# onecodex/needletail

Measured on AMD Instinct MI355X. Metric: Gbases/s canonical k=21 on 150 bp FASTQ; % HBM-read roofline at 1/2/4/8 GPU, higher is better.
Workload: dtype u64; 1 GPU; configs[1]: synthetic FASTQ 10M x 150 bp, k=21 canonical k-mers (normalize -> reverse_complement -> canonical_kmers), reduce mode, device-resident batch; reads_total=10000000, reads_this_gpu=10000000, read_len=150, k=21, seed=0x5eed0002, outputs=n_total,n_fwd,n_rc,4096-bin prefix histogram,sum64,xor64, parallelism=single GPU, rccl_ranks=0, devices_visible=1

## Files before the change

include/needletail_amd.h:

```cpp
#ifndef NEEDLETAIL_AMD_H
#define NEEDLETAIL_AMD_H

#include <stddef.h>
#include <stdint.h>

#ifdef __cplusplus
extern "C" {
#endif

#define NTK_ABI_VERSION 4

enum {
    NTK_OK = 0,
    NTK_ERR_BAD_K = 1,
    NTK_ERR_BAD_ARG = 2,
    NTK_ERR_HIP = 3,
    NTK_ERR_NO_DEVICE = 4,
    NTK_ERR_CAPACITY = 5,
    NTK_ERR_UNSUPPORTED = 6,
    NTK_ERR_NOMEM = 7,
    NTK_ERR_PARSE = 8,
    NTK_ERR_RCCL = 9,
    NTK_EOF = 100
};
// ... 35 lines not shown
    uint64_t hist[NTK_HIST_BINS];
    uint64_t n_undigested;
} ntk_result;
#define NTK_ACC_N_TOTAL 0
#define NTK_ACC_N_FWD 1
#define NTK_ACC_N_RC 2
#define NTK_ACC_SUM 3
#define NTK_ACC_XOR 4
#define NTK_ACC_UNDIGESTED 5
#define NTK_ACC_REDONE 6
#define NTK_ACC_HIST 8
#define NTK_ACC_XOR_BITS (8 + NTK_HIST_BINS)
#define NTK_ACC_WORDS (8 + NTK_HIST_BINS + 64)

typedef struct ntk_ctx ntk_ctx;
int ntk_ctx_create(int device, ntk_ctx **out);
int ntk_ctx_create_on_stream(int device, void *hip_stream, ntk_ctx **out);
void ntk_ctx_destroy(ntk_ctx *ctx);
int ntk_ctx_synchronize(ntk_ctx *ctx);
int ntk_ctx_stream(ntk_ctx *ctx, int *device, void **hip_stream);
int ntk_ctx_set_launch(ntk_ctx *ctx, int blocks, int threads_per_block);
enum { NTK_OPT_COMPAT_CHUNK_BYTES = 1, NTK_OPT_MINIMIZER_CHUNK_BYTES = 2, NTK_OPT_MINIMIZER_ROUTE = 3, NTK_OPT_COMPAT_PACK_THREADS = 4,
       NTK_OPT_COPY_STREAMS = 5, NTK_OPT_BATCH_WAIT_POLL_US = 6, NTK_OPT_GZ_INMEM_LIMIT_BYTES = 7, NTK_OPT_GZ_STREAM_WINDOW_BYTES = 8,
       NTK_OPT_PIPE_STATS = 9 };
#define NTK_POLL_BLOCK 0xFFFFFFFFu
#define NTK_ROUTE_NO_REGFUSED 1u
#define NTK_ROUTE_NO_GENERIC 2u
#define NTK_ROUTE_NO_F64 4u
#define NTK_ROUTE_NO_SPECULATION 8u
int ntk_ctx_set_option(ntk_ctx *ctx, int option, uint64_t value);
int ntk_ctx_get_option(ntk_ctx *ctx, int option, uint64_t *value);
int ntk_ctx_enable_timing(ntk_ctx *ctx, int on);
int ntk_ctx_scan_time_ms(ntk_ctx *ctx, double *total_ms, uint64_t *launches);

typedef struct ntk_comm ntk_comm;
#define NTK_COMM_ID_BYTES 128
int ntk_comm_init_all(ntk_ctx *const *ctxs, int n, ntk_comm **out);
int ntk_comm_unique_id(uint8_t id[NTK_COMM_ID_BYTES]);
int ntk_comm_init_rank(ntk_ctx *ctx, int n_ranks, int rank, const uint8_t id[NTK_COMM_ID_BYTES], ntk_comm **out);
int ntk_comm_size(const ntk_comm *comm);
int ntk_allreduce_accumulators(ntk_comm *comm);
int ntk_comm_allreduce_time_ms(ntk_comm *comm, double *total_ms, uint64_t *calls);
void ntk_comm_destroy(ntk_comm *comm);

int ntk_accum_reset(ntk_ctx *ctx);
int ntk_reduce_device(ntk_ctx *ctx, const uint8_t *d_seq, uint64_t n_bytes, const ntk_params *p);
int ntk_reduce_device_quality(ntk_ctx *ctx, const uint8_t *d_seq, const uint8_t *d_qual, uint64_t n_bytes,
// ... 108 lines not shown
```

needletail_amd/_lib.py:

```python
from __future__ import annotations

import ctypes as C
import os

_HERE = os.path.dirname(os.path.abspath(__file__))
LIB_PATH = os.environ.get("NEEDLETAIL_AMD_LIB") or os.path.join(_HERE, "libneedletail_amd.so")

NTK_OK = 0
PATH_BYTES_CANONICAL, PATH_BITS, PATH_BITS_CANONICAL = 0, 1, 2
PRE_NONE, PRE_STRIP_RETURNS, PRE_NORMALIZE, PRE_NORMALIZE_IUPAC = 0, 1, 2, 3
HIST_BINS = 4096
ACC_N_TOTAL, ACC_N_FWD, ACC_N_RC, ACC_SUM, ACC_XOR, ACC_HIST = 0, 1, 2, 3, 4, 8
ACC_UNDIGESTED, ACC_REDONE = 5, 6
ACC_XOR_BITS, ACC_WORDS = 8 + 4096, 8 + 4096 + 64
OPT_COMPAT_CHUNK_BYTES, OPT_MINIMIZER_CHUNK_BYTES, OPT_MINIMIZER_ROUTE, OPT_COMPAT_PACK_THREADS, OPT_COPY_STREAMS = 1, 2, 3, 4, 5
OPT_BATCH_WAIT_POLL_US, OPT_GZ_INMEM_LIMIT_BYTES, OPT_GZ_STREAM_WINDOW_BYTES, OPT_PIPE_STATS = 6, 7, 8, 9
POLL_BLOCK = 0xFFFFFFFF
ROUTE_NO_REGFUSED, ROUTE_NO_GENERIC, ROUTE_NO_F64, ROUTE_NO_SPECULATION = 1, 2, 4, 8
ROUTE_TWO_PASS = ROUTE_NO_REGFUSED | ROUTE_NO_GENERIC

SYMBOLS = [
    "ntk_strerror", "ntk_last_hip_error", "ntk_last_rccl_error", "ntk_abi_version", "ntk_device_count",
    "ntk_comm_init_all", "ntk_comm_unique_id", "ntk_comm_init_rank", "ntk_comm_size", "ntk_allreduce_accumulators", "ntk_comm_allreduce_time_ms", "ntk_comm_destroy",
    "ntk_ctx_create", "ntk_ctx_create_on_stream", "ntk_ctx_destroy", "ntk_ctx_synchronize", "ntk_ctx_stream",
    "ntk_ctx_set_launch", "ntk_ctx_set_option", "ntk_ctx_get_option", "ntk_ctx_enable_timing", "ntk_ctx_scan_time_ms",
    "ntk_accum_reset", "ntk_reduce_device", "ntk_reduce_device_quality", "ntk_accum_read", "ntk_accum_device_ptr", "ntk_accum_bind_device",
    "ntk_materialize_device", "ntk_materialize_device_quality",
    "ntk_batch_acquire", "ntk_batch_append", "ntk_batch_append_quality", "ntk_batch_buffers", "ntk_batch_submit", "ntk_batch_wait",
    "ntk_batch_release",
    "ntk_normalize", "ntk_strip_returns", "ntk_reverse_complement", "ntk_canonical_kmers", "ntk_bit_kmers", "ntk_canonical_kmers_batch", "ntk_bit_kmers_batch", "ntk_pinned_alloc", "ntk_pinned_free",
    "ntk_canonical_kmers_batch_planes", "ntk_bit_kmers_batch_planes", "ntk_ctx_trim", "ntk_minimizer_batch",
    "ntk_synth_reads_device", "ntk_reverse_complement_records_device",
    "ntk_reader_open_file", "ntk_reader_open_memory", "ntk_reader_next", "ntk_reader_error", "ntk_reader_position", "ntk_reader_close",
    "ntk_scan_reader", "ntk_scan_buffer_parallel", "ntk_scan_file_parallel", "ntk_fastx_split_points", "ntk_gunzip", "ntk_gunzip_free", "ntk_scan_file_info",
    "ntk_minimizers_reduce_device", "ntk_minimizer", "ntk_canonical", "ntk_bit_minimizers", "ntk_quality_mask", "ntk_bit_canonical",
]


class Params(C.Structure):
# ... 158 lines not shown
```

needletail_amd/csrc/ntk_api.hip:

```cpp
#include "../../include/needletail_amd.h"

#include <hip/hip_runtime.h>
#include <rccl/rccl.h>
#include <dlfcn.h>
#include <time.h>

#include <cstdlib>
#include <cstring>
#include <map>
#include <mutex>
#include <new>
#include <utility>
#include <thread>
#include <algorithm>
#include <vector>

#include "ntk_kernels.hpp"

using namespace ntk;

const void *ntk_pick_scan2(int k, bool tie_rc, bool accept_u);
const void *ntk_pick_scan2_q(int k, bool canonical, bool tie_rc, bool accept_u);
const void *ntk_pick_scan2_min_a(int k, int w, bool tie_rc, bool accept_u, bool quality);
const void *ntk_pick_scan2_min_b(int k, int w, bool tie_rc, bool accept_u, bool quality);
// ... 72 lines not shown

struct ntk_ctx {
    int device = 0;
    hipStream_t stream = nullptr;
    hipStream_t copy_stream = nullptr;
    hipStream_t copy_stream2 = nullptr;
    uint32_t copy_streams = 2, copy_rr = 0;
    hipStream_t down_stream = nullptr;
    bool owns_stream = false;
    int n_cu = 256;
    int launch_blocks = 0, launch_threads = 0;
    uint64_t *d_acc = nullptr;
    uint64_t *d_acc_own = nullptr;
    uint32_t *d_part_hist = nullptr;
    uint32_t *d_work = nullptr;
    bool work_dirty = true;
    uint32_t *d_lower = nullptr;
    uint32_t lower_idx = 0;
    uint64_t minimizer_chunk = (uint64_t)256 << 20;
    uint64_t compat_chunk = (uint64_t)16 << 20;
    uint32_t route_off = 0;
    uint32_t pack_threads = 8;
    uint64_t wait_poll_us = 50;
    uint64_t gz_limit = 0, gz_window = 0, pipe_stats = 0;
    uint64_t *d_part_scalars = nullptr;
    int part_blocks = 0;
    uint16_t *d_lut = nullptr;
    Scratch scratch[6];
    CompatBank bank[3];
    void *h_pinned = nullptr;
    bool timing = false;
    std::vector<hipEvent_t> ev_free;
    std::vector<std::pair<hipEvent_t, hipEvent_t>> ev_used;
    std::map<std::pair<const void *, int>, int> occupancy;
    std::map<const void *, int> auto_threads;
    std::mutex pool_mu;
    std::vector<ntk_batch *> pool;
    uint64_t pool_bytes = 0;
};

struct ntk_batch {
    uint8_t *h_seq = nullptr;
    uint64_t *h_off = nullptr;
    uint8_t *d_seq = nullptr;
    uint8_t *h_qual = nullptr, *d_qual = nullptr;
    bool has_qual = false;
// ... 240 lines not shown
int launch_tile_scan(ntk_ctx *c, const TileScan &s, ScanArgs &a, bool zero_first)
{
    int per_cu = 0, rc = resident_blocks(c, s.fn, s.threads, s.lds, s.max_per_cu, &per_cu);
    if (rc) return rc;
    const uint64_t blocks_max = block_cap(c, per_cu), waves_per_block = (uint64_t)s.threads / 64;
    const uint64_t tile_slots = 64 - (uint64_t)s.halo_lanes, tile_stride = tile_slots * 16, n = a.n_bytes;
    const int blocks_raw = s.speculate ? raw_bytes_blocks(c, n) : 0;
    a.n_tiles = tile_count(n, tile_slots);
    a.work_counters = c->d_work;
    a.zero_words = NTK_ACC_WORDS;
    for (uint64_t tb = 0; tb < a.n_tiles; tb += kMaxTilesPerLaunch) {
        const uint64_t te = tb + kMaxTilesPerLaunch < a.n_tiles ? tb + kMaxTilesPerLaunch : a.n_tiles;
        const uint64_t tiles = te - tb;
        uint64_t chunk = tiles / (blocks_max * waves_per_block * 4);
        chunk = chunk < 1 ? 1 : (chunk > s.max_chunk ? s.max_chunk : chunk);
        const uint64_t want_blocks = (tiles + chunk * waves_per_block - 1) / (chunk * waves_per_block);
        const int blocks = (int)(want_blocks < blocks_max ? want_blocks : blocks_max);
        a.tile_begin = tb; a.tile_end = te;
        const uint64_t first_tail = n / tile_stride;
        a.tail_tile_rel = first_tail < tb ? 0u : (first_tail - tb > 0xFFFFFFFEull ? 0xFFFFFFFFu : (uint32_t)(first_tail - tb));
        a.n_shards = blocks < kMaxShards ? (uint32_t)blocks : (uint32_t)kMaxShards;
        a.tiles_per_shard = (uint32_t)((tiles + a.n_shards - 1) / a.n_shards);
        a.chunk_tiles = (uint32_t)chunk;
        a.zero_acc = zero_first ? c->d_acc : nullptr;
        zero_first = false;
        if (c->work_dirty) HIPCHK(hipMemsetAsync(c->d_work, 0, kMaxShards * 64, c->stream));
        c->work_dirty = true;
        if (s.reduce) {
            if ((rc = ensure_partials(c, blocks > blocks_raw ? blocks : blocks_raw))) return rc;
            a.part_hist = c->d_part_hist; a.part_scalars = c->d_part_scalars;
        }
        Fold fold;
        fold.rearm_shards = a.n_shards;
        if (s.speculate) {
            const FlagPair f = next_flag(c);
            a.lower_flag = f.flag; a.lower_flag_next = f.next;
            fold.alt_flag = f.flag; fold.alt_rows = blocks_raw;
        }
        TimedSpan span;
        if ((rc = span.begin(c))) return rc;
        void *kargs[] = {(void *)&a};
        HIPCHK(hipLaunchKernel(s.fn, dim3(blocks), dim3(s.threads), kargs, s.lds, c->stream));
        if (s.speculate) {
            launch_raw_bytes(c, false, blocks_raw, a.seq, n, a.k, fold.alt_flag, false, a.qual, s.cutoff);
            HIPCHK(hipGetLastError());
        }
// ... 241 lines not shown
    return NTK_OK;
}

int ntk_ctx_set_launch(ntk_ctx *c, int blocks, int threads)
{
    if (!c || blocks < 0 || threads < 0 || threads > 1024 || (threads & 63)) return NTK_ERR_BAD_ARG;
    c->launch_blocks = blocks; c->launch_threads = threads;
    return NTK_OK;
}

int ntk_ctx_get_option(ntk_ctx *c, int option, uint64_t *value)
{
    if (!c || !value) return NTK_ERR_BAD_ARG;
    switch (option) {
    case NTK_OPT_COMPAT_CHUNK_BYTES: *value = c->compat_chunk; return NTK_OK;
    case NTK_OPT_MINIMIZER_CHUNK_BYTES: *value = c->minimizer_chunk; return NTK_OK;
    case NTK_OPT_MINIMIZER_ROUTE: *value = c->route_off; return NTK_OK;
    case NTK_OPT_COMPAT_PACK_THREADS: *value = c->pack_threads; return NTK_OK;
    case NTK_OPT_COPY_STREAMS: *value = c->copy_streams; return NTK_OK;
    case NTK_OPT_BATCH_WAIT_POLL_US: *value = c->wait_poll_us ? c->wait_poll_us : NTK_POLL_BLOCK; return NTK_OK;
    case NTK_OPT_GZ_INMEM_LIMIT_BYTES: *value = c->gz_limit; return NTK_OK;
    case NTK_OPT_GZ_STREAM_WINDOW_BYTES: *value = c->gz_window; return NTK_OK;
    case NTK_OPT_PIPE_STATS: *value = c->pipe_stats; return NTK_OK;
    default: return NTK_ERR_BAD_ARG;
    }
}

int ntk_ctx_set_option(ntk_ctx *c, int option, uint64_t value)
{
    if (!c) return NTK_ERR_BAD_ARG;
    switch (option) {
    case NTK_OPT_COMPAT_CHUNK_BYTES:
        c->compat_chunk = value == 0 ? ((uint64_t)16 << 20) : (value < 64 ? 64 : value);
        return NTK_OK;
    case NTK_OPT_MINIMIZER_CHUNK_BYTES:
        if (value && value < 4096) return NTK_ERR_BAD_ARG;
        c->minimizer_chunk = value == 0 ? ((uint64_t)256 << 20) : (value & ~(uint64_t)4095);
        return NTK_OK;
    case NTK_OPT_MINIMIZER_ROUTE:
        if (value & ~(uint64_t)(NTK_ROUTE_NO_REGFUSED | NTK_ROUTE_NO_GENERIC | NTK_ROUTE_NO_F64 | NTK_ROUTE_NO_SPECULATION)) return NTK_ERR_BAD_ARG;
        c->route_off = (uint32_t)value;
        return NTK_OK;
    case NTK_OPT_BATCH_WAIT_POLL_US:
        c->wait_poll_us = value == 0 ? 50 : (value == NTK_POLL_BLOCK ? 0 : (value > 10000000 ? 10000000 : value));
        return NTK_OK;
    case NTK_OPT_GZ_INMEM_LIMIT_BYTES: c->gz_limit = value; return NTK_OK;
// ... 1208 lines not shown
```

needletail_amd/csrc/ntk_kernels.hpp:

```cpp
#pragma once
#include <hip/hip_runtime.h>
#include <stdint.h>
#include <type_traits>

#include "ntk_tile.hpp"

#if !defined(NTK_KBENCH) && (defined(NTK_ABL_LOADSONLY) || defined(NTK_ABL_FLOOR) || defined(NTK_ABL_NOLDS) || defined(NTK_ABL_NODIGEST) || \
                             defined(NTK_ABL_NOEXEC) || defined(NTK_ABL_NOSDWA) || defined(NTK_ABL_NOMASKALG) || defined(NTK_V_CLOCKS) || \
                             defined(NTK_X_CMPFIRST) || defined(NTK_X_TWOPHASE) || defined(NTK_X_MFMASUM) || defined(NTK_X_SELOUT) || defined(NTK_X_PREFETCH2) || defined(NTK_X_FASTSTART) || defined(NTK_ABL_HALFIMPORTS))
#error "NTK_ABL_* / NTK_X_* / NTK_V_CLOCKS are kernel-bench switches: build with -DNTK_KBENCH (tools/build_kbench.sh), never into the library"
#endif

namespace ntk {

typedef uint32_t u32x4 __attribute__((ext_vector_type(4)));

constexpr int kDppWaveShr1 = 0x138;
struct DevXL {
    __device__ __forceinline__ uint32_t prev_and(int s, uint32_t x, uint32_t mask) const { return prev(s, x) & mask; }
    __device__ __forceinline__ uint32_t prev_auto(uint32_t x) const { return prev(0, x); }
    __device__ __forceinline__ uint32_t prev(int, uint32_t x) const
    {
        return (uint32_t)__builtin_amdgcn_mov_dpp((int)x, kDppWaveShr1, 0xf, 0xf, true);
    }
    __device__ __forceinline__ uint32_t prev_add(int, uint32_t x, uint32_t c) const
    {
        uint32_t r;
        asm("s_nop 1\n v_add_u32_dpp %0, %1, %2 wave_shr:1 row_mask:0xf bank_mask:0xf bound_ctrl:1" : "=v"(r) : "v"(x), "v"(c));
        return r;
    }
    __device__ __forceinline__ uint32_t select_prev(int, bool take, uint32_t a, uint32_t b) const
    {
// ... 562 lines not shown
#define NTK_SV2_MINWAVES 1
#endif
template <int K, bool TIE_RC, bool ACCEPT_U, bool QM = false, int HB = 12, int W = 0, bool FWD = false>
__global__ __launch_bounds__(1024, NTK_SV2_MINWAVES) void scan2_kernel(ScanArgs a)
{
    static_assert(K >= 1 && K <= 32 && (HB == 12 || HB == 14), "sv2 covers 1 <= k <= 32");
    static_assert(W == 0 || Sv2MinFused<K, W>::value, "fused minimizers: see ntk_tile.hpp");
    static_assert(W == 0 || K <= 16 || Sv2Light<K, HB>::value, "fused minimizers sum the lo word only: the cell must cover the bits above it");
    constexpr bool WORD = K <= 16;
    constexpr bool LIGHT = Sv2Light<K, HB>::value && !WORD;
    constexpr int kCells = 1 << HB;
    using Geo = Sv2Geom<(W ? K + W - 1 : K)>;
    constexpr uint32_t kStride = Geo::kStride, kHaloB = Geo::kHaloBytes;
    struct Lds { uint32_t hist[kCells]; uint64_t red[16 * 6]; };
    __shared__ Lds L;
    uint32_t *const s_hist = L.hist;
    uint64_t *const s_red = L.red;
    if ((uint32_t)(uintptr_t)&L.hist[0] != 0u) __builtin_trap();

#ifdef NTK_V_CLOCKS
    const uint64_t dbg_c0 = clock64(), dbg_w0 = wall_clock64();
    uint32_t dbg_tiles = 0;
#endif
#ifndef NTK_X_FASTSTART
    if (a.zero_acc && blockIdx.x == 0)
        for (uint32_t i = threadIdx.x; i < a.zero_words; i += blockDim.x) a.zero_acc[i] = 0;
    for (int i = threadIdx.x; i < kCells; i += blockDim.x) s_hist[i] = 0;
    __syncthreads();

#endif
    const uint32_t lane = threadIdx.x & 63u;
    const uint32_t wave = __builtin_amdgcn_readfirstlane(threadIdx.x >> 6);
    const uint32_t shard = blockIdx.x % a.n_shards;
    const uint32_t launch_tiles = (uint32_t)(a.tile_end - a.tile_begin);
    const uint32_t shard_begin = shard * a.tiles_per_shard;
    uint32_t shard_end = shard_begin + a.tiles_per_shard;
    if (shard_end > launch_tiles) shard_end = launch_tiles;
    uint32_t *ctr = a.work_counters + shard * 16;
    const uint32_t shard_tiles = shard_begin < shard_end ? shard_end - shard_begin : 0u;
#ifdef NTK_X_FASTSTART
    uint32_t next = 0;
    if (lane == 0) next = atomicAdd(ctr, a.chunk_tiles);
    if (a.zero_acc && blockIdx.x == 0)
        for (uint32_t i = threadIdx.x; i < a.zero_words; i += blockDim.x) a.zero_acc[i] = 0;
    for (int i = threadIdx.x; i < kCells / 4; i += blockDim.x) reinterpret_cast<u32x4 *>(s_hist)[i] = u32x4{0u, 0u, 0u, 0u};
    __syncthreads();
#endif
    constexpr bool SPEC = TIE_RC && !ACCEPT_U && W == 0 && !FWD;
    uint32_t lc = 0;
    if (SPEC && a.lower_flag_next && blockIdx.x == 0 && threadIdx.x == 0) *a.lower_flag_next = 0;
    DevXL xl;
    DevMasks2<K, HB> mp;
    NoSink sink;
    mp.rep = lane & (uint32_t)(DevMasks2<K, HB>::kWordCopies - 1);
#ifdef NTK_X_MFMASUM
    { const int sel = 1 << (8 * (lane & 3)); mp.msel = {sel, sel, sel, sel}; }
#endif

#ifndef NTK_X_FASTSTART
    uint32_t next = 0;
    if (lane == 0) next = atomicAdd(ctr, a.chunk_tiles);
#endif
    next = __builtin_amdgcn_readfirstlane(next);
#ifdef NTK_X_GUIDED
    uint32_t c_cur = a.chunk_tiles;
    const uint32_t shard_waves2 = 2u * ((gridDim.x + a.n_shards - 1) / a.n_shards) * (blockDim.x >> 6);
#endif
    while (next < shard_tiles) {
        const uint32_t r0 = shard_begin + next;
#ifdef NTK_X_GUIDED
        uint32_t r1 = r0 + c_cur;
        if (r1 > shard_end) r1 = shard_end;
        {
            const uint32_t done = next + c_cur < shard_tiles ? next + c_cur : shard_tiles;
            uint32_t c = (shard_tiles - done) / shard_waves2;
            c = c < 2u ? 2u : (c > a.chunk_tiles ? a.chunk_tiles : c);
            c_cur = c;
            if (lane == 0) next = atomicAdd(ctr, c);
        }
#else
        uint32_t r1 = r0 + a.chunk_tiles;
        if (r1 > shard_end) r1 = shard_end;
        if (lane == 0) next = atomicAdd(ctr, a.chunk_tiles);
#endif
        const uint64_t t0 = a.tile_begin + r0;
        const uint64_t run_byte = t0 * kStride;
        const uint32_t halo = t0 ? kHaloB : 0u;
        const uint64_t cbase = (uint64_t)a.seq + run_byte - halo;
        uint64_t rem = ((a.n_bytes + 15) & ~(uint64_t)15) - (run_byte - halo);
        if (rem > 0xFFFFFF00ull) rem = 0xFFFFFF00ull;
        const uint32_t blo = __builtin_amdgcn_readfirstlane((uint32_t)cbase);
        const uint32_t bhi = __builtin_amdgcn_readfirstlane((uint32_t)(cbase >> 32));
        const uint32_t nrec = __builtin_amdgcn_readfirstlane((uint32_t)rem);
        __amdgpu_buffer_rsrc_t rs = __builtin_amdgcn_make_buffer_rsrc((void *)(((uint64_t)bhi << 32) | blo), 0, nrec, 0x00020000);
        __amdgpu_buffer_rsrc_t rq = rs;
        if constexpr (QM) {
            const uint64_t qbase = (uint64_t)a.qual + run_byte - halo;
            const uint32_t qlo = __builtin_amdgcn_readfirstlane((uint32_t)qbase);
            const uint32_t qhi = __builtin_amdgcn_readfirstlane((uint32_t)(qbase >> 32));
            rq = __builtin_amdgcn_make_buffer_rsrc((void *)(((uint64_t)qhi << 32) | qlo), 0, nrec, 0x00020000);
        }
        uint32_t voff = lane * 16u - (kHaloB - halo);
        uint64_t tile_byte = run_byte;
#ifdef NTK_ABL_FLOOR
        auto load_tile = [&](uint32_t off) { (void)rs; return u32x4{off, off, off, off}; };
#else
        auto load_tile = [&](uint32_t off) { return __builtin_amdgcn_raw_buffer_load_b128(rs, off, 0, 0); };
#endif
        auto load_qual = [&](uint32_t off) { return __builtin_amdgcn_raw_buffer_load_b128(rq, off, 0, 0); };
#ifdef NTK_ABL_FLOOR
        uint32_t fl_code = lane * 0x9E3779B9u + r0, fl_rcode = ~fl_code, fl_step = 0x85EBCA6Bu + lane;
        asm volatile("" : "+v"(fl_step));
#pragma unroll
        for (int i = 0; i < 16; i++) { mp.VA[i] = ~3ull; mp.VB[i] = ~0ull; }
#endif
        auto process = [&](const u32x4 &t, const u32x4 &q, uint32_t r, auto &&after_encode) {
            const bool tail = r >= a.tail_tile_rel;
            Raw16 raw{t.x, t.y, t.z, t.w};
            if constexpr (SPEC && !QM) {
                if (tail) lc |= or_of_input_bytes(raw, (int64_t)a.n_bytes - ((int64_t)tile_byte - (int64_t)kHaloB + lane * 16));
                else lc = bitop3<0xFE>(bitop3<0xFE>(lc, t.x, t.y), t.z, t.w);
            }
            if constexpr (QM) raw = quality_break16(raw, Raw16{q.x, q.y, q.z, q.w}, a.q_add, a.q_sel);
            if constexpr (SPEC && QM) {
                if (tail) lc |= or_of_input_bytes(lower_watch16(raw), (int64_t)a.n_bytes - ((int64_t)tile_byte - (int64_t)kHaloB + lane * 16));
                else lc = lower_watch_or(lower_watch_or(lower_watch_or(lower_watch_or(lc, raw.x), raw.y), raw.z), raw.w);
            }
#ifdef NTK_ABL_LOADSONLY
            mp.xlo ^= raw.x ^ raw.y ^ raw.z ^ raw.w; (void)tail;
            after_encode();
#elif defined(NTK_ABL_FLOOR)
            (void)tail; (void)raw;
            after_encode();
            fl_code += fl_step; fl_rcode += fl_code;
            lane_tile_sv2<TIE_RC, K>(sink, xl, mp, fl_code, fl_rcode);
#else
            const EncSV2 en = encode16_sv2<ACCEPT_U>(raw);
            mp.template compute<(W ? K + W - 1 : K)>(en, tail, (int64_t)tile_byte - (int64_t)kHaloB + lane * 16, a.n_bytes);
            after_encode();
            if constexpr (W > 0) lane_tile_sv2_min<TIE_RC, K, W>(sink, xl, mp, en.code, en.rcode);
            else if constexpr (WORD) lane_tile_sv2w<TIE_RC, K, FWD>(sink, xl, mp, en.code, en.rcode);
            else if constexpr (FWD) lane_tile_sv2_fwd<K>(sink, xl, mp, en.code);
            else lane_tile_sv2<TIE_RC, K>(sink, xl, mp, en.code, en.rcode);
#endif
            voff += kStride; tile_byte += kStride;
#ifdef NTK_V_CLOCKS
            dbg_tiles++;
#endif
        };
        u32x4 ta = load_tile(voff), qa = ta;
        if constexpr (QM) qa = load_qual(voff);
#ifdef NTK_X_PREFETCH2
        u32x4 tb = ta;
        if (r0 + 1 < r1) tb = load_tile(voff + kStride);
        for (uint32_t r = r0; r < r1; r += 2) {
            process(ta, qa, r, [&] { if (r + 2 < r1) ta = load_tile(voff + 2 * kStride); });
            if (r + 1 < r1) process(tb, qa, r + 1, [&] { if (r + 3 < r1) tb = load_tile(voff + 2 * kStride); });
        }
#else
        for (uint32_t r = r0; r < r1; r++)
            process(ta, qa, r, [&] {
                if (r + 1 < r1) { ta = load_tile(voff + kStride); if constexpr (QM) qa = load_qual(voff + kStride); }
            });
#endif
        next = __builtin_amdgcn_readfirstlane(next);
    }

#ifdef NTK_V_CLOCKS
    if ((threadIdx.x & 63) == 0 && a.values) {
        uint32_t hwid, xcc;
        asm volatile("s_getreg_b32 %0, hwreg(HW_REG_HW_ID)" : "=s"(hwid));
        asm volatile("s_getreg_b32 %0, hwreg(HW_REG_XCC_ID)" : "=s"(xcc));
        const size_t w = (size_t)blockIdx.x * (blockDim.x >> 6) + (threadIdx.x >> 6);
        a.values[w * 4 + 0] = dbg_w0; a.values[w * 4 + 1] = wall_clock64();
        a.values[w * 4 + 2] = ((clock64() - dbg_c0) & 0xFFFFFFFFFFull) | ((uint64_t)dbg_tiles << 40); a.values[w * 4 + 3] = ((uint64_t)xcc << 32) | hwid;
    }
#endif
    if constexpr (SPEC)
        if (a.lower_flag && __builtin_amdgcn_ballot_w64((lc & 0x20202020u) != 0u) != 0ull && lane == 0) atomicOr(a.lower_flag, 1u);
    asm volatile("s_waitcnt lgkmcnt(0)" ::: "memory");
    uint64_t sum = mp.sum + mp.sum2 + ((uint64_t)mp.sumh << 32);
#ifdef NTK_X_MFMASUM
    if ((lane & 15) < 4) sum += (uint64_t)(int64_t)(mp.macc.x + mp.macc.y + mp.macc.z + mp.macc.w) << (8 * (lane & 3));
#endif
    uint64_t xr = (WORD || LIGHT) ? (uint64_t)mp.xlo : ((uint64_t)mp.xh << 32) | mp.xlo, nf, nv = 0;
    uint64_t shi = 0, xf = 0;
    uint32_t *ph = a.part_hist + (size_t)blockIdx.x * kHistBins;
    nf = lane == 0 ? mp.nf_s : 0u;
    if constexpr (W > 0) nf = mp.nf_bits;
    __syncthreads();
    constexpr int HBE = HB;
    for (int c = threadIdx.x; c < kHistBins; c += blockDim.x) {
        uint32_t tot = 0;
        if constexpr (K <= 6) {
            if (c < (1 << (2 * K)))
                for (int r = 0; r < DevMasks2<K, HB>::kWordCopies; r++) tot += s_hist[(r << (2 * K)) + c];
        } else
#pragma unroll
        for (int q = 0; q < kCells / kHistBins; q++) {
            const uint32_t f = c * (kCells / kHistBins) + q, h = s_hist[f];
            tot += h;
            if constexpr (LIGHT) {
                const uint32_t pfx = f >> (HB - HBE);
                shi += (uint64_t)(pfx >> (32 + HBE - 2 * K)) * h;
                xf ^= (h & 1u) ? pfx : 0u;
            }
        }
        ph[c] = tot; nv += tot;
    }
    if constexpr (LIGHT) {
        constexpr uint32_t low_mask = 2 * K - HBE >= 32 ? 0xFFFFFFFFu : ((1u << ((2 * K - HBE) & 31)) - 1u);
        sum += shi << 32;
        xr = (xf << (2 * K - HBE)) | (uint64_t)(mp.xlo & low_mask);
    }
#pragma unroll
    for (int o = 32; o > 0; o >>= 1) {
        sum += __shfl_xor(sum, o, 64);
        xr ^= __shfl_xor(xr, o, 64);
        nf += __shfl_xor(nf, o, 64);
        nv += __shfl_xor(nv, o, 64);
    }
    if (lane == 0) { s_red[wave * 4 + 0] = nv; s_red[wave * 4 + 1] = nf; s_red[wave * 4 + 2] = sum; s_red[wave * 4 + 3] = xr; }
    __syncthreads();
    if (threadIdx.x == 0) {
        uint64_t tv = 0, tf = 0, ts = 0, tx = 0;
        for (uint32_t w = 0; w < (blockDim.x >> 6); w++) {
            tv += s_red[w * 4 + 0]; tf += s_red[w * 4 + 1]; ts += s_red[w * 4 + 2]; tx ^= s_red[w * 4 + 3];
        }
        uint64_t *ps = a.part_scalars + (size_t)blockIdx.x * 4;
        if constexpr (W > 0 && !TIE_RC) tf = tv - tf;
        if constexpr (FWD) tf = tv;
        if constexpr (WORD && K < 16 && W == 0) { ts >>= 32 - 2 * K; tx >>= 32 - 2 * K; }
        ps[0] = tv; ps[1] = tf; ps[2] = ts; ps[3] = tx;
    }
}

#ifndef NTK_SCAN_TEMPLATES_ONLY
#ifndef NTK_MINGEN_WAVES_F64
#define NTK_MINGEN_WAVES_F64 4
#endif
#ifndef NTK_MINGEN_WAVES_G
#define NTK_MINGEN_WAVES_G 4
#endif
constexpr int min_gen_waves(bool f64) { return f64 ? NTK_MINGEN_WAVES_F64 : NTK_MINGEN_WAVES_G; }
constexpr int min_gen_threads(bool f64) { return min_gen_waves(f64) == 3 ? 768 : 512; }
struct DevMinOut {
    uint64_t sum = 0, sum2 = 0;
    uint32_t sumh = 0, xh = 0;
    uint32_t xlo = 0, nfb = 0, one = 1;
    template <bool WIDE>
    __device__ __forceinline__ void region(const uint64_t *V, const uint32_t (&off)[4], const uint32_t (&lo)[4], const uint32_t (&hi)[4],
                                           const uint32_t (&sb)[4])
    {
        uint64_t sd;
#define NTK_M_POS(i, ACC, W)                                                \
        "s_mov_b64 exec, %[m" #i "]\n"                                      \
// ... 154 lines not shown
                if (light) { shi += (uint64_t)(f >> (46u - 2u * kk)) * h; xf ^= (h & 1u) ? f : 0u; }
            }
        ph[c] = tot;
    }
    if (light) {
        const uint32_t low_bits = 2u * kk - 14u;
        sum += shi << 32;
        xr = (xf << low_bits) | (low_bits >= 32u ? xr : (xr & ((1ull << low_bits) - 1ull)));
    }
#pragma unroll
    for (int o = 32; o > 0; o >>= 1) {
        sum += __shfl_xor(sum, o, 64); xr ^= __shfl_xor(xr, o, 64); nf += __shfl_xor(nf, o, 64); nv += __shfl_xor(nv, o, 64);
    }
    if (lane == 0) { s_red[wave * 4 + 0] = nv; s_red[wave * 4 + 1] = nf; s_red[wave * 4 + 2] = sum; s_red[wave * 4 + 3] = xr; }
    __syncthreads();
    if (threadIdx.x == 0) {
        uint64_t tv = 0, tf = 0, ts = 0, tx = 0;
        for (uint32_t w = 0; w < (blockDim.x >> 6); w++) { tv += s_red[w * 4 + 0]; tf += s_red[w * 4 + 1]; ts += s_red[w * 4 + 2]; tx ^= s_red[w * 4 + 3]; }
        uint64_t *ps = a.part_scalars + (size_t)blockIdx.x * 4;
        ps[0] = tv; ps[1] = tf; ps[2] = ts; ps[3] = tx;
    }
}

constexpr int kFoldThreads = 256, kFoldBinGroups = kHistBins / kFoldThreads, kFoldRowGroups = 32;
constexpr int kFoldBlocks = kFoldBinGroups * kFoldRowGroups + 1;
__global__ __launch_bounds__(kFoldThreads) void fold_kernel(const uint32_t *part_hist, const uint64_t *part_scalars, int nblocks,
                                                            uint64_t *acc, uint32_t *work_counters = nullptr, int n_counters = 8,
                                                            const uint32_t *select = nullptr, int nblocks_alt = 0, int undigested = 0)
{
    if (select && *select) nblocks = nblocks_alt;
    if (blockIdx.x < kFoldBinGroups * kFoldRowGroups) {
        const int bin = (blockIdx.x % kFoldBinGroups) * kFoldThreads + threadIdx.x;
        uint64_t s = 0;
#pragma unroll 8
        for (int b = blockIdx.x / kFoldBinGroups; b < nblocks; b += kFoldRowGroups) s += part_hist[(size_t)b * kHistBins + bin];
        if (s) atomicAdd((unsigned long long *)&acc[8 + bin], (unsigned long long)s);
        return;
    }
    __shared__ uint64_t s_red[kFoldThreads / 64][4];
    if (work_counters)
        for (int i = threadIdx.x; i < n_counters; i += kFoldThreads) work_counters[i * 16] = 0;
    uint64_t tv = 0, tf = 0, ts = 0, tx = 0;
    for (int b = threadIdx.x; b < nblocks; b += kFoldThreads) {
        tv += part_scalars[b * 4 + 0]; tf += part_scalars[b * 4 + 1];
        ts += part_scalars[b * 4 + 2]; tx ^= part_scalars[b * 4 + 3];
    }
#pragma unroll
    for (int o = 32; o > 0; o >>= 1) {
        tv += __shfl_xor(tv, o, 64); tf += __shfl_xor(tf, o, 64); ts += __shfl_xor(ts, o, 64); tx ^= __shfl_xor(tx, o, 64);
    }
    if ((threadIdx.x & 63) == 0) { s_red[threadIdx.x >> 6][0] = tv; s_red[threadIdx.x >> 6][1] = tf; s_red[threadIdx.x >> 6][2] = ts; s_red[threadIdx.x >> 6][3] = tx; }
    __syncthreads();
    if (threadIdx.x < 64) {
        tv = tf = ts = tx = 0;
        for (int w = 0; w < kFoldThreads / 64; w++) { tv += s_red[w][0]; tf += s_red[w][1]; ts += s_red[w][2]; tx ^= s_red[w][3]; }
        if (threadIdx.x == 0) {
            acc[0] += tv; acc[1] += tf; acc[2] += tv - tf; acc[3] += ts; acc[4] ^= tx;
            if (undigested) acc[5] += tv;
            if (select && *select) acc[6] += 1;
        }
        acc[8 + kHistBins + threadIdx.x] += (tx >> threadIdx.x) & 1;
    }
}


template <int THREADS, class T>
__device__ __forceinline__ T block_exclusive_scan(T v, T *s_wave, T *total = nullptr)
{
    T x = v;
#pragma unroll
    for (int o = 1; o < 64; o <<= 1) {
        const T y = __shfl_up(x, o, 64);
        if ((int)(threadIdx.x & 63) >= o) x += y;
    }
    __syncthreads();
    if ((threadIdx.x & 63) == 63) s_wave[threadIdx.x >> 6] = x;
    __syncthreads();
    T wave_off = 0, all = 0;
#pragma unroll
    for (int w = 0; w < THREADS / 64; w++) {
        const T t = s_wave[w];
        if (w < (int)(threadIdx.x >> 6)) wave_off += t;
        all += t;
    }
// ... 901 lines not shown
```

Measured before the change: 3231 Gbases/s.

## Statically assign first scan chunks per wave, defer LDS zeroing, restructure fold kernel

Each wave now takes its first chunk from a fixed offset based on its shard rank instead of an atomic, and later atomic pulls are offset by a pull base. The tile load for the first chunk is issued before the LDS histogram is zeroed, so the two can overlap. The histogram epilogue reads LDS with 128-bit loads and writes partials with relaxed atomic stores. The fold kernel uses fewer row groups, keeps 16 rows of 128-bit loads in flight per wave, combines waves through LDS, and reads the scalar accumulators early. Together these aim to cut startup and atomic contention and raise memory-level parallelism in the fold, at the cost of more complex work-distribution logic that must stay consistent with the counter reset.

Result: no change. 3256 Gbases/s (median of 2 runs) (+0.8%).

```diff
diff --git a/include/needletail_amd.h b/include/needletail_amd.h
--- a/include/needletail_amd.h
+++ b/include/needletail_amd.h
@@ -81,7 +81,7 @@
 int ntk_ctx_set_launch(ntk_ctx *ctx, int blocks, int threads_per_block);
 enum { NTK_OPT_COMPAT_CHUNK_BYTES = 1, NTK_OPT_MINIMIZER_CHUNK_BYTES = 2, NTK_OPT_MINIMIZER_ROUTE = 3, NTK_OPT_COMPAT_PACK_THREADS = 4,
        NTK_OPT_COPY_STREAMS = 5, NTK_OPT_BATCH_WAIT_POLL_US = 6, NTK_OPT_GZ_INMEM_LIMIT_BYTES = 7, NTK_OPT_GZ_STREAM_WINDOW_BYTES = 8,
-       NTK_OPT_PIPE_STATS = 9 };
+       NTK_OPT_PIPE_STATS = 9, NTK_OPT_LAST_SCAN_WAVES = 10, NTK_OPT_LAST_SCAN_CHUNK_TILES = 11 };
 #define NTK_POLL_BLOCK 0xFFFFFFFFu
 #define NTK_ROUTE_NO_REGFUSED 1u
 #define NTK_ROUTE_NO_GENERIC 2u
diff --git a/needletail_amd/_lib.py b/needletail_amd/_lib.py
--- a/needletail_amd/_lib.py
+++ b/needletail_amd/_lib.py
@@ -15,6 +15,7 @@
 ACC_XOR_BITS, ACC_WORDS = 8 + 4096, 8 + 4096 + 64
 OPT_COMPAT_CHUNK_BYTES, OPT_MINIMIZER_CHUNK_BYTES, OPT_MINIMIZER_ROUTE, OPT_COMPAT_PACK_THREADS, OPT_COPY_STREAMS = 1, 2, 3, 4, 5
 OPT_BATCH_WAIT_POLL_US, OPT_GZ_INMEM_LIMIT_BYTES, OPT_GZ_STREAM_WINDOW_BYTES, OPT_PIPE_STATS = 6, 7, 8, 9
+OPT_LAST_SCAN_WAVES, OPT_LAST_SCAN_CHUNK_TILES = 10, 11
 POLL_BLOCK = 0xFFFFFFFF
 ROUTE_NO_REGFUSED, ROUTE_NO_GENERIC, ROUTE_NO_F64, ROUTE_NO_SPECULATION = 1, 2, 4, 8
 ROUTE_TWO_PASS = ROUTE_NO_REGFUSED | ROUTE_NO_GENERIC
diff --git a/needletail_amd/csrc/ntk_api.hip b/needletail_amd/csrc/ntk_api.hip
--- a/needletail_amd/csrc/ntk_api.hip
+++ b/needletail_amd/csrc/ntk_api.hip
@@ -118,6 +118,7 @@
     uint32_t route_off = 0;
     uint32_t pack_threads = 8;
     uint64_t wait_poll_us = 50;
+    uint64_t last_scan_waves = 0, last_scan_chunk = 0;
     uint64_t gz_limit = 0, gz_window = 0, pipe_stats = 0;
     uint64_t *d_part_scalars = nullptr;
     int part_blocks = 0;
@@ -404,6 +405,7 @@
         a.n_shards = blocks < kMaxShards ? (uint32_t)blocks : (uint32_t)kMaxShards;
         a.tiles_per_shard = (uint32_t)((tiles + a.n_shards - 1) / a.n_shards);
         a.chunk_tiles = (uint32_t)chunk;
+        c->last_scan_waves = (uint64_t)blocks * waves_per_block; c->last_scan_chunk = chunk;
         a.zero_acc = zero_first ? c->d_acc : nullptr;
         zero_first = false;
         if (c->work_dirty) HIPCHK(hipMemsetAsync(c->d_work, 0, kMaxShards * 64, c->stream));
@@ -691,6 +693,8 @@
     case NTK_OPT_GZ_INMEM_LIMIT_BYTES: *value = c->gz_limit; return NTK_OK;
     case NTK_OPT_GZ_STREAM_WINDOW_BYTES: *value = c->gz_window; return NTK_OK;
     case NTK_OPT_PIPE_STATS: *value = c->pipe_stats; return NTK_OK;
+    case NTK_OPT_LAST_SCAN_WAVES: *value = c->last_scan_waves; return NTK_OK;
+    case NTK_OPT_LAST_SCAN_CHUNK_TILES: *value = c->last_scan_chunk; return NTK_OK;
     default: return NTK_ERR_BAD_ARG;
     }
 }
diff --git a/needletail_amd/csrc/ntk_kernels.hpp b/needletail_amd/csrc/ntk_kernels.hpp
--- a/needletail_amd/csrc/ntk_kernels.hpp
+++ b/needletail_amd/csrc/ntk_kernels.hpp
@@ -7,7 +7,7 @@
 
 #if !defined(NTK_KBENCH) && (defined(NTK_ABL_LOADSONLY) || defined(NTK_ABL_FLOOR) || defined(NTK_ABL_NOLDS) || defined(NTK_ABL_NODIGEST) || \
                              defined(NTK_ABL_NOEXEC) || defined(NTK_ABL_NOSDWA) || defined(NTK_ABL_NOMASKALG) || defined(NTK_V_CLOCKS) || \
-                             defined(NTK_X_CMPFIRST) || defined(NTK_X_TWOPHASE) || defined(NTK_X_MFMASUM) || defined(NTK_X_SELOUT) || defined(NTK_X_PREFETCH2) || defined(NTK_X_FASTSTART) || defined(NTK_ABL_HALFIMPORTS))
+                             defined(NTK_X_CMPFIRST) || defined(NTK_X_TWOPHASE) || defined(NTK_X_MFMASUM) || defined(NTK_X_SELOUT) || defined(NTK_X_PREFETCH2) || defined(NTK_X_OLDSTART) || defined(NTK_X_PLAINROWS) || defined(NTK_ABL_HALFIMPORTS))
 #error "NTK_ABL_* / NTK_X_* / NTK_V_CLOCKS are kernel-bench switches: build with -DNTK_KBENCH (tools/build_kbench.sh), never into the library"
 #endif
 
@@ -616,29 +616,24 @@
     const uint64_t dbg_c0 = clock64(), dbg_w0 = wall_clock64();
     uint32_t dbg_tiles = 0;
 #endif
-#ifndef NTK_X_FASTSTART
-    if (a.zero_acc && blockIdx.x == 0)
-        for (uint32_t i = threadIdx.x; i < a.zero_words; i += blockDim.x) a.zero_acc[i] = 0;
-    for (int i = threadIdx.x; i < kCells; i += blockDim.x) s_hist[i] = 0;
-    __syncthreads();
-
-#endif
     const uint32_t lane = threadIdx.x & 63u;
     const uint32_t wave = __builtin_amdgcn_readfirstlane(threadIdx.x >> 6);
-    const uint32_t shard = blockIdx.x % a.n_shards;
+    const uint32_t shard_rank = blockIdx.x / a.n_shards, shard = blockIdx.x - shard_rank * a.n_shards;
     const uint32_t launch_tiles = (uint32_t)(a.tile_end - a.tile_begin);
     const uint32_t shard_begin = shard * a.tiles_per_shard;
     uint32_t shard_end = shard_begin + a.tiles_per_shard;
     if (shard_end > launch_tiles) shard_end = launch_tiles;
     uint32_t *ctr = a.work_counters + shard * 16;
     const uint32_t shard_tiles = shard_begin < shard_end ? shard_end - shard_begin : 0u;
-#ifdef NTK_X_FASTSTART
-    uint32_t next = 0;
-    if (lane == 0) next = atomicAdd(ctr, a.chunk_tiles);
-    if (a.zero_acc && blockIdx.x == 0)
-        for (uint32_t i = threadIdx.x; i < a.zero_words; i += blockDim.x) a.zero_acc[i] = 0;
-    for (int i = threadIdx.x; i < kCells / 4; i += blockDim.x) reinterpret_cast<u32x4 *>(s_hist)[i] = u32x4{0u, 0u, 0u, 0u};
-    __syncthreads();
+    auto zero_block = [&] {
+        if (a.zero_acc && blockIdx.x == 0)
+            for (uint32_t i = threadIdx.x; i < a.zero_words; i += blockDim.x) a.zero_acc[i] = 0;
+        for (int i = threadIdx.x; i < kCells / 4; i += blockDim.x) reinterpret_cast<u32x4 *>(s_hist)[i] = u32x4{0u, 0u, 0u, 0u};
+        asm volatile("s_waitcnt lgkmcnt(0)\n"
+                     "s_barrier" ::: "memory");
+    };
+#ifdef NTK_X_OLDSTART
+    zero_block();
 #endif
     constexpr bool SPEC = TIE_RC && !ACCEPT_U && W == 0 && !FWD;
     uint32_t lc = 0;
@@ -651,32 +646,39 @@
     { const int sel = 1 << (8 * (lane & 3)); mp.msel = {sel, sel, sel, sel}; }
 #endif
 
-#ifndef NTK_X_FASTSTART
+    const uint32_t block_waves = blockDim.x >> 6;
+#ifdef NTK_X_OLDSTART
+    const uint32_t pull_base = 0;
     uint32_t next = 0;
     if (lane == 0) next = atomicAdd(ctr, a.chunk_tiles);
-#endif
     next = __builtin_amdgcn_readfirstlane(next);
+#else
+    const uint32_t pull_base = ((gridDim.x - 1u - shard) / a.n_shards + 1u) * block_waves * a.chunk_tiles;
+    uint32_t next = (shard_rank * block_waves + wave) * a.chunk_tiles;
+#endif
 #ifdef NTK_X_GUIDED
     uint32_t c_cur = a.chunk_tiles;
-    const uint32_t shard_waves2 = 2u * ((gridDim.x + a.n_shards - 1) / a.n_shards) * (blockDim.x >> 6);
-#endif
-    while (next < shard_tiles) {
-        const uint32_t r0 = shard_begin + next;
-#ifdef NTK_X_GUIDED
-        uint32_t r1 = r0 + c_cur;
-        if (r1 > shard_end) r1 = shard_end;
-        {
-            const uint32_t done = next + c_cur < shard_tiles ? next + c_cur : shard_tiles;
-            uint32_t c = (shard_tiles - done) / shard_waves2;
-            c = c < 2u ? 2u : (c > a.chunk_tiles ? a.chunk_tiles : c);
-            c_cur = c;
-            if (lane == 0) next = atomicAdd(ctr, c);
-        }
+    const uint32_t shard_waves2 = 2u * ((gridDim.x + a.n_shards - 1) / a.n_shards) * block_waves;
+#endif
+    uint32_t r0 = 0, r1 = 0, voff = 0;
+    uint64_t tile_byte = 0;
+    __amdgpu_buffer_rsrc_t rs = __builtin_amdgcn_make_buffer_rsrc((void *)a.seq, 0, 0, 0x00020000), rq = rs;
+    u32x4 ta = {0u, 0u, 0u, 0u}, qa = ta;
+#ifdef NTK_ABL_FLOOR
+    auto load_tile = [&](uint32_t off) { (void)rs; return u32x4{off, off, off, off}; };
 #else
-        uint32_t r1 = r0 + a.chunk_tiles;
-        if (r1 > shard_end) r1 = shard_end;
-        if (lane == 0) next = atomicAdd(ctr, a.chunk_tiles);
-#endif
+    auto load_tile = [&](uint32_t off) { return __builtin_amdgcn_raw_buffer_load_b128(rs, off, 0, 0); };
+#endif
+    auto load_qual = [&](uint32_t off) { return __builtin_amdgcn_raw_buffer_load_b128(rq, off, 0, 0); };
+#ifdef NTK_ABL_FLOOR
+    uint32_t fl_code = 0, fl_rcode = 0, fl_step = 0x85EBCA6Bu + lane;
+    asm volatile("" : "+v"(fl_step));
+#endif
+    auto begin_chunk = [&](uint32_t first_tile, uint32_t chunk) {
+        r0 = shard_begin + first_tile;
+        uint32_t last_tile = first_tile + chunk;
+        if (last_tile > shard_tiles) last_tile = shard_tiles;
+        r1 = shard_begin + last_tile;
         const uint64_t t0 = a.tile_begin + r0;
         const uint64_t run_byte = t0 * kStride;
         const uint32_t halo = t0 ? kHaloB : 0u;
@@ -686,64 +688,75 @@
         const uint32_t blo = __builtin_amdgcn_readfirstlane((uint32_t)cbase);
         const uint32_t bhi = __builtin_amdgcn_readfirstlane((uint32_t)(cbase >> 32));
         const uint32_t nrec = __builtin_amdgcn_readfirstlane((uint32_t)rem);
-        __amdgpu_buffer_rsrc_t rs = __builtin_amdgcn_make_buffer_rsrc((void *)(((uint64_t)bhi << 32) | blo), 0, nrec, 0x00020000);
-        __amdgpu_buffer_rsrc_t rq = rs;
+        rs = __builtin_amdgcn_make_buffer_rsrc((void *)(((uint64_t)bhi << 32) | blo), 0, nrec, 0x00020000);
+        rq = rs;
         if constexpr (QM) {
             const uint64_t qbase = (uint64_t)a.qual + run_byte - halo;
             const uint32_t qlo = __builtin_amdgcn_readfirstlane((uint32_t)qbase);
             const uint32_t qhi = __builtin_amdgcn_readfirstlane((uint32_t)(qbase >> 32));
             rq = __builtin_amdgcn_make_buffer_rsrc((void *)(((uint64_t)qhi << 32) | qlo), 0, nrec, 0x00020000);
         }
-        uint32_t voff = lane * 16u - (kHaloB - halo);
-        uint64_t tile_byte = run_byte;
+        voff = lane * 16u - (kHaloB - halo);
+        tile_byte = run_byte;
 #ifdef NTK_ABL_FLOOR
-        auto load_tile = [&](uint32_t off) { (void)rs; return u32x4{off, off, off, off}; };
+        fl_code = lane * 0x9E3779B9u + r0; fl_rcode = ~fl_code;
+#pragma unroll
+        for (int i = 0; i < 16; i++) { mp.VA[i] = ~3ull; mp.VB[i] = ~0ull; }
+#endif
+        ta = load_tile(voff); qa = ta;
+        if constexpr (QM) qa = load_qual(voff);
+    };
+    auto process = [&](const u32x4 &t, const u32x4 &q, uint32_t r, auto &&after_encode) {
+        const bool tail = r >= a.tail_tile_rel;
+        Raw16 raw{t.x, t.y, t.z, t.w};
+        if constexpr (SPEC && !QM) {
+            if (tail) lc |= or_of_input_bytes(raw, (int64_t)a.n_bytes - ((int64_t)tile_byte - (int64_t)kHaloB + lane * 16));
+            else lc = bitop3<0xFE>(bitop3<0xFE>(lc, t.x, t.y), t.z, t.w);
+        }
+        if constexpr (QM) raw = quality_break16(raw, Raw16{q.x, q.y, q.z, q.w}, a.q_add, a.q_sel);
+        if constexpr (SPEC && QM) {
+            if (tail) lc |= or_of_input_bytes(lower_watch16(raw), (int64_t)a.n_bytes - ((int64_t)tile_byte - (int64_t)kHaloB + lane * 16));
+            else lc = lower_watch_or(lower_watch_or(lower_watch_or(lower_watch_or(lc, raw.x), raw.y), raw.z), raw.w);
+        }
+#ifdef NTK_ABL_LOADSONLY
+        mp.xlo ^= raw.x ^ raw.y ^ raw.z ^ raw.w; (void)tail;
+        after_encode();
+#elif defined(NTK_ABL_FLOOR)
+        (void)tail; (void)raw;
+        after_encode();
+        fl_code += fl_step; fl_rcode += fl_code;
+        lane_tile_sv2<TIE_RC, K>(sink, xl, mp, fl_code, fl_rcode);
 #else
-        auto load_tile = [&](uint32_t off) { return __builtin_amdgcn_raw_buffer_load_b128(rs, off, 0, 0); };
-#endif
-        auto load_qual = [&](uint32_t off) { return __builtin_amdgcn_raw_buffer_load_b128(rq, off, 0, 0); };
-#ifdef NTK_ABL_FLOOR
-        uint32_t fl_code = lane * 0x9E3779B9u + r0, fl_rcode = ~fl_code, fl_step = 0x85EBCA6Bu + lane;
-        asm volatile("" : "+v"(fl_step));
-#pragma unroll
-        for (int i = 0; i < 16; i++) { mp.VA[i] = ~3ull; mp.VB[i] = ~0ull; }
-#endif
-        auto process = [&](const u32x4 &t, const u32x4 &q, uint32_t r, auto &&after_encode) {
-            const bool tail = r >= a.tail_tile_rel;
-            Raw16 raw{t.x, t.y, t.z, t.w};
-            if constexpr (SPEC && !QM) {
-                if (tail) lc |= or_of_input_bytes(raw, (int64_t)a.n_bytes - ((int64_t)tile_byte - (int64_t)kHaloB + lane * 16));
-                else lc = bitop3<0xFE>(bitop3<0xFE>(lc, t.x, t.y), t.z, t.w);
-            }
-            if constexpr (QM) raw = quality_break16(raw, Raw16{q.x, q.y, q.z, q.w}, a.q_add, a.q_sel);
-            if constexpr (SPEC && QM) {
-                if (tail) lc |= or_of_input_bytes(lower_watch16(raw), (int64_t)a.n_bytes - ((int64_t)tile_byte - (int64_t)kHaloB + lane * 16));
-                else lc = lower_watch_or(lower_watch_or(lower_watch_or(lower_watch_or(lc, raw.x), raw.y), raw.z), raw.w);
-            }
-#ifdef NTK_ABL_LOADSONLY
-            mp.xlo ^= raw.x ^ raw.y ^ raw.z ^ raw.w; (void)tail;
-            after_encode();
-#elif defined(NTK_ABL_FLOOR)
-            (void)tail; (void)raw;
-            after_encode();
-            fl_code += fl_step; fl_rcode += fl_code;
-            lane_tile_sv2<TIE_RC, K>(sink, xl, mp, fl_code, fl_rcode);
+        const EncSV2 en = encode16_sv2<ACCEPT_U>(raw);
+        mp.template compute<(W ? K + W - 1 : K)>(en, tail, (int64_t)tile_byte - (int64_t)kHaloB + lane * 16, a.n_bytes);
+        after_encode();
+        if constexpr (W > 0) lane_tile_sv2_min<TIE_RC, K, W>(sink, xl, mp, en.code, en.rcode);
+        else if constexpr (WORD) lane_tile_sv2w<TIE_RC, K, FWD>(sink, xl, mp, en.code, en.rcode);
+        else if constexpr (FWD) lane_tile_sv2_fwd<K>(sink, xl, mp, en.code);
+        else lane_tile_sv2<TIE_RC, K>(sink, xl, mp, en.code, en.rcode);
+#endif
+        voff += kStride; tile_byte += kStride;
+#ifdef NTK_V_CLOCKS
+        dbg_tiles++;
+#endif
+    };
+    bool have = next < shard_tiles;
+    if (have) begin_chunk(next, a.chunk_tiles);
+#ifndef NTK_X_OLDSTART
+    zero_block();
+#endif
+    while (have) {
+#ifdef NTK_X_GUIDED
+        {
+            const uint32_t done = next + c_cur < shard_tiles ? next + c_cur : shard_tiles;
+            uint32_t c = (shard_tiles - done) / shard_waves2;
+            c = c < 2u ? 2u : (c > a.chunk_tiles ? a.chunk_tiles : c);
+            c_cur = c;
+            if (lane == 0) next = atomicAdd(ctr, c);
+        }
 #else
-            const EncSV2 en = encode16_sv2<ACCEPT_U>(raw);
-            mp.template compute<(W ? K + W - 1 : K)>(en, tail, (int64_t)tile_byte - (int64_t)kHaloB + lane * 16, a.n_bytes);
-            after_encode();
-            if constexpr (W > 0) lane_tile_sv2_min<TIE_RC, K, W>(sink, xl, mp, en.code, en.rcode);
-            else if constexpr (WORD) lane_tile_sv2w<TIE_RC, K, FWD>(sink, xl, mp, en.code, en.rcode);
-            else if constexpr (FWD) lane_tile_sv2_fwd<K>(sink, xl, mp, en.code);
-            else lane_tile_sv2<TIE_RC, K>(sink, xl, mp, en.code, en.rcode);
-#endif
-            voff += kStride; tile_byte += kStride;
-#ifdef NTK_V_CLOCKS
-            dbg_tiles++;
-#endif
-        };
-        u32x4 ta = load_tile(voff), qa = ta;
-        if constexpr (QM) qa = load_qual(voff);
+        if (lane == 0) next = atomicAdd(ctr, a.chunk_tiles);
+#endif
 #ifdef NTK_X_PREFETCH2
         u32x4 tb = ta;
         if (r0 + 1 < r1) tb = load_tile(voff + kStride);
@@ -757,7 +770,13 @@
                 if (r + 1 < r1) { ta = load_tile(voff + kStride); if constexpr (QM) qa = load_qual(voff + kStride); }
             });
 #endif
-        next = __builtin_amdgcn_readfirstlane(next);
+        next = __builtin_amdgcn_readfirstlane(next) + pull_base;
+        have = next < shard_tiles;
+#ifdef NTK_X_GUIDED
+        if (have) begin_chunk(next, c_cur);
+#else
+        if (have) begin_chunk(next, a.chunk_tiles);
+#endif
     }
 
 #ifdef NTK_V_CLOCKS
@@ -789,10 +808,17 @@
         if constexpr (K <= 6) {
             if (c < (1 << (2 * K)))
                 for (int r = 0; r < DevMasks2<K, HB>::kWordCopies; r++) tot += s_hist[(r << (2 * K)) + c];
+        } else {
+        uint32_t cells[kCells / kHistBins];
+        if constexpr (kCells / kHistBins == 4) {
+            const u32x4 h4 = reinterpret_cast<const u32x4 *>(s_hist)[c];
+            cells[0] = h4.x; cells[1] = h4.y; cells[2] = h4.z; cells[3] = h4.w;
         } else
 #pragma unroll
+        for (int q = 0; q < kCells / kHistBins; q++) cells[q] = s_hist[c * (kCells / kHistBins) + q];
+#pragma unroll
         for (int q = 0; q < kCells / kHistBins; q++) {
-            const uint32_t f = c * (kCells / kHistBins) + q, h = s_hist[f];
+            const uint32_t f = c * (kCells / kHistBins) + q, h = cells[q];
             tot += h;
             if constexpr (LIGHT) {
                 const uint32_t pfx = f >> (HB - HBE);
@@ -800,7 +826,13 @@
                 xf ^= (h & 1u) ? pfx : 0u;
             }
         }
-        ph[c] = tot; nv += tot;
+        }
+#ifdef NTK_X_PLAINROWS
+        ph[c] = tot;
+#else
+        __hip_atomic_store(&ph[c], tot, __ATOMIC_RELAXED, __HIP_MEMORY_SCOPE_AGENT);
+#endif
+        nv += tot;
     }
     if constexpr (LIGHT) {
         constexpr uint32_t low_mask = 2 * K - HBE >= 32 ? 0xFFFFFFFFu : ((1u << ((2 * K - HBE) & 31)) - 1u);
@@ -825,7 +857,13 @@
         if constexpr (W > 0 && !TIE_RC) tf = tv - tf;
         if constexpr (FWD) tf = tv;
         if constexpr (WORD && K < 16 && W == 0) { ts >>= 32 - 2 * K; tx >>= 32 - 2 * K; }
-        ps[0] = tv; ps[1] = tf; ps[2] = ts; ps[3] = tx;
+        const uint64_t out[4] = {tv, tf, ts, tx};
+#pragma unroll
+#ifdef NTK_X_PLAINROWS
+        for (int i = 0; i < 4; i++) ps[i] = out[i];
+#else
+        for (int i = 0; i < 4; i++) __hip_atomic_store(&ps[i], out[i], __ATOMIC_RELAXED, __HIP_MEMORY_SCOPE_AGENT);
+#endif
     }
 }
 
@@ -1026,25 +1064,53 @@
     }
 }
 
-constexpr int kFoldThreads = 256, kFoldBinGroups = kHistBins / kFoldThreads, kFoldRowGroups = 32;
+constexpr int kFoldThreads = 256, kFoldBinGroups = kHistBins / kFoldThreads, kFoldRowGroups = 8, kFoldRowsInFlight = 16;
 constexpr int kFoldBlocks = kFoldBinGroups * kFoldRowGroups + 1;
+static_assert(kFoldThreads == 256 && kHistBins % kFoldThreads == 0, "a fold wave covers 256 bins with 128-bit loads");
 __global__ __launch_bounds__(kFoldThreads) void fold_kernel(const uint32_t *part_hist, const uint64_t *part_scalars, int nblocks,
                                                             uint64_t *acc, uint32_t *work_counters = nullptr, int n_counters = 8,
                                                             const uint32_t *select = nullptr, int nblocks_alt = 0, int undigested = 0)
 {
-    if (select && *select) nblocks = nblocks_alt;
-    if (blockIdx.x < kFoldBinGroups * kFoldRowGroups) {
-        const int bin = (blockIdx.x % kFoldBinGroups) * kFoldThreads + threadIdx.x;
-        uint64_t s = 0;
-#pragma unroll 8
-        for (int b = blockIdx.x / kFoldBinGroups; b < nblocks; b += kFoldRowGroups) s += part_hist[(size_t)b * kHistBins + bin];
-        if (s) atomicAdd((unsigned long long *)&acc[8 + bin], (unsigned long long)s);
+    const bool alt = select && *select;
+    if (alt) nblocks = nblocks_alt;
+    if (blockIdx.x > 0) {
+        constexpr int kWaves = kFoldThreads / 64, kRowStep = kFoldRowGroups * kWaves, kRowQuads = kHistBins / 4;
+        __shared__ uint64_t s_bins[kWaves][kFoldThreads];
+        const int piece = blockIdx.x - 1, bin_group = piece % kFoldBinGroups, wave = threadIdx.x >> 6, lane = threadIdx.x & 63;
+        const u32x4 *col = reinterpret_cast<const u32x4 *>(part_hist) + bin_group * (kFoldThreads / 4) + lane;
+        uint64_t s[4] = {0, 0, 0, 0};
+        for (int b0 = (piece / kFoldBinGroups) * kWaves + wave; b0 < nblocks; b0 += kRowStep * kFoldRowsInFlight) {
+            u32x4 v[kFoldRowsInFlight];
+#pragma unroll
+            for (int i = 0; i < kFoldRowsInFlight; i++) {
+                const int b = b0 + i * kRowStep;
+                v[i] = col[(size_t)(b < nblocks ? b : nblocks - 1) * kRowQuads];
+            }
+#pragma unroll
+            for (int i = 0; i < kFoldRowsInFlight; i++)
+                if (b0 + i * kRowStep < nblocks) { s[0] += v[i].x; s[1] += v[i].y; s[2] += v[i].z; s[3] += v[i].w; }
+        }
+#pragma unroll
+        for (int j = 0; j < 4; j++) s_bins[wave][lane * 4 + j] = s[j];
+        __syncthreads();
+        uint64_t tot = 0;
+#pragma unroll
+        for (int w = 0; w < kWaves; w++) tot += s_bins[w][threadIdx.x];
+        if (tot) atomicAdd((unsigned long long *)&acc[8 + bin_group * kFoldThreads + threadIdx.x], (unsigned long long)tot);
         return;
     }
     __shared__ uint64_t s_red[kFoldThreads / 64][4];
+    uint64_t old[6] = {0, 0, 0, 0, 0, 0}, old_redone = 0, old_bit = 0;
+    if (threadIdx.x == 0) {
+#pragma unroll
+        for (int i = 0; i < 6; i++) old[i] = acc[i];
+        old_redone = acc[6];
+    }
+    if (threadIdx.x < 64) old_bit = acc[8 + kHistBins + threadIdx.x];
     if (work_counters)
         for (int i = threadIdx.x; i < n_counters; i += kFoldThreads) work_counters[i * 16] = 0;
     uint64_t tv = 0, tf = 0, ts = 0, tx = 0;
+#pragma unroll 2
     for (int b = threadIdx.x; b < nblocks; b += kFoldThreads) {
         tv += part_scalars[b * 4 + 0]; tf += part_scalars[b * 4 + 1];
         ts += part_scalars[b * 4 + 2]; tx ^= part_scalars[b * 4 + 3];
@@ -1059,11 +1125,11 @@
         tv = tf = ts = tx = 0;
         for (int w = 0; w < kFoldThreads / 64; w++) { tv += s_red[w][0]; tf += s_red[w][1]; ts += s_red[w][2]; tx ^= s_red[w][3]; }
         if (threadIdx.x == 0) {
-            acc[0] += tv; acc[1] += tf; acc[2] += tv - tf; acc[3] += ts; acc[4] ^= tx;
-            if (undigested) acc[5] += tv;
-            if (select && *select) acc[6] += 1;
-        }
-        acc[8 + kHistBins + threadIdx.x] += (tx >> threadIdx.x) & 1;
+            acc[0] = old[0] + tv; acc[1] = old[1] + tf; acc[2] = old[2] + (tv - tf); acc[3] = old[3] + ts; acc[4] = old[4] ^ tx;
+            if (undigested) acc[5] = old[5] + tv;
+            if (alt) acc[6] = old_redone + 1;
+        }
+        acc[8 + kHistBins + threadIdx.x] = old_bit + ((tx >> threadIdx.x) & 1);
     }
 }
 
```
